# Tamnemng/TAM-GCN

Measured on AMD Instinct MI355X. Metric: skeleton clips/sec (fwd+CE+bwd+grad all-reduce+SGD step), N-UCLA 20-joint x 64-frame, higher is better.
Workload: dtype f32 (exact fp32-input MFMA v_mfma_f32_16x16x4_f32 in every GEMM, forward and backward: the reference's arithmetic); 1 GPU; N-UCLA joint stream, 256 clips/GPU x (3,64,20,1), models.ctrgcn.Model fwd+CE+bwd+grad-allreduce+SGD step, train-mode BN; global_batch=256, streams=1, parallelism=dp1, launch=hipgraph, model_streams=0, rehearsal=False, allreduce=one flat bucket after backward

## Files before the change

### include/tamgcn.h

```cpp
#ifndef TAMGCN_H
#define TAMGCN_H

#ifdef __cplusplus
extern "C" {
#endif

#define TAMGCN_VERSION 401
#define TAMGCN_MAX_SUBSETS 3
#define TAMGCN_MAX_V 32

typedef struct tamgcn_src {
    const float* x1;
    const float* x2;
    const float* coef;
    int ctot;
    int coff;
    int act;
} tamgcn_src;

int         tamgcn_version(void);
const char* tamgcn_last_error(void);
const char* tamgcn_last_kernel(void);
int         tamgcn_get_split_mode(void);
int         tamgcn_set_split_mode(int mode);
// ... 20 lines not shown
    const tamgcn_src* mask;
    const float* aux;
    const float* aux_center;
    int auxctot, auxcoff;
    float* stats_part;
    int stats_ctot, stats_coff;
    const float* post_coef;
    int post_ctot, post_act;
} tamgcn_conv_desc;

int tamgcn_conv_nparts(const tamgcn_conv_desc* d);
int tamgcn_conv(const tamgcn_conv_desc* d, void* stream);

typedef struct tamgcn_wgrad_desc {
    tamgcn_src gy;
    tamgcn_src src;
    int N, M, K, T_in, T_out, V, KT, dil, stride, pad;
    float* part;
    int nsplit;
} tamgcn_wgrad_desc;
int tamgcn_wgrad_max_split(const tamgcn_wgrad_desc* d);
int tamgcn_wgrad(const tamgcn_wgrad_desc* d, void* stream);

typedef struct tamgcn_reduce_desc {
    const float* part; float* out;
    int nsplit, accumulate;
    long long stride_s, count;
    float scale;
} tamgcn_reduce_desc;
int tamgcn_reduce_multi(const tamgcn_reduce_desc* descs, int n, void* stream);

int tamgcn_reduce_sum(float* part, int nsplit, long long stride_s, long long count,
                      float scale, int accumulate, float* out, void* stream);

int tamgcn_bn_fwd_finalize(const float* part, int part_ctot, int part_coff, int nparts, double count,
                           const float* gamma, const float* beta,
                           float* running_mean, float* running_var, long long* num_batches_tracked,
                           float momentum, float eps, int training,
                           float* coef, float* save, int coef_ctot, int coef_coff, int C, void* stream);

int tamgcn_coef_diff(const float* coef_d, const float* coef_y, float* out, int C, int mode, void* stream);

int tamgcn_bn_bwd_finalize(const float* part, int part_ctot, int part_coff, int nparts, double count,
                           const float* gamma, const float* save, int save_ctot, int save_coff,
                           int training, float* dgamma, float* dbeta, float* dbias_conv,
                           float* coef, int coef_ctot, int coef_coff, int C, void* stream);
// ... 222 lines not shown
```

### tam_gcn_amd/_lib.py

```python
import ctypes as C
import os

_HERE = os.path.dirname(os.path.abspath(__file__))
LIB_PATH = os.path.join(_HERE, 'libtamgcn.so')

c_float_p = C.c_void_p


class Src(C.Structure):
    _fields_ = [('x1', C.c_void_p), ('x2', C.c_void_p), ('coef', C.c_void_p),
                ('ctot', C.c_int), ('coff', C.c_int), ('act', C.c_int)]


class ConvDesc(C.Structure):
    _fields_ = [('src', Src),
                ('N', C.c_int), ('K', C.c_int), ('T_in', C.c_int), ('V', C.c_int),
                ('w', C.c_void_p), ('bias', C.c_void_p),
                ('M', C.c_int), ('KT', C.c_int), ('dil', C.c_int), ('stride', C.c_int), ('pad', C.c_int),
                ('wmode', C.c_int), ('up', C.c_int),
                ('y', C.c_void_p), ('yctot', C.c_int), ('ycoff', C.c_int),
                ('T_out', C.c_int), ('T_y', C.c_int), ('ostride', C.c_int),
                ('add1', C.c_void_p), ('add2', C.c_void_p), ('bcast', C.c_void_p), ('bcast_scale', C.c_float),
                ('mask', C.POINTER(Src)),
                ('aux', C.c_void_p), ('aux_center', C.c_void_p), ('auxctot', C.c_int), ('auxcoff', C.c_int),
# ... 1 lines not shown
                ('post_coef', C.c_void_p), ('post_ctot', C.c_int), ('post_act', C.c_int)]


TCONV_MAXB = 6


class TconvDesc(C.Structure):
    _fields_ = [('src', Src),
                ('N', C.c_int), ('T_in', C.c_int), ('T_out', C.c_int), ('V', C.c_int), ('Cb', C.c_int), ('nb', C.c_int),
                ('KT', C.c_int), ('stride', C.c_int), ('pool', C.c_int),
                ('dil', C.c_int * TCONV_MAXB), ('w', C.c_void_p * TCONV_MAXB), ('bias', C.c_void_p * TCONV_MAXB),
                ('y', C.c_void_p), ('yctot', C.c_int), ('ycoff', C.c_int),
                ('stats_part', C.c_void_p), ('stats_ctot', C.c_int),
                ('mask', C.POINTER(Src)), ('center', C.c_void_p)]


class WgradDesc(C.Structure):
    _fields_ = [('gy', Src), ('src', Src),
                ('N', C.c_int), ('M', C.c_int), ('K', C.c_int), ('T_in', C.c_int), ('T_out', C.c_int),
                ('V', C.c_int), ('KT', C.c_int), ('dil', C.c_int), ('stride', C.c_int), ('pad', C.c_int),
                ('part', C.c_void_p), ('nsplit', C.c_int)]


class ReduceDesc(C.Structure):
    _fields_ = [('part', C.c_void_p), ('out', C.c_void_p), ('nsplit', C.c_int), ('accumulate', C.c_int),
                ('stride_s', C.c_longlong), ('count', C.c_longlong), ('scale', C.c_float)]


class BnFwdDesc(C.Structure):
    _fields_ = [('part', C.c_void_p), ('part_ctot', C.c_int), ('part_coff', C.c_int), ('nparts', C.c_int), ('count', C.c_double),
                ('gamma', C.c_void_p), ('beta', C.c_void_p), ('running_mean', C.c_void_p), ('running_var', C.c_void_p),
                ('num_batches_tracked', C.c_void_p), ('momentum', C.c_float), ('eps', C.c_float), ('training', C.c_int),
                ('coef', C.c_void_p), ('save', C.c_void_p), ('coef_ctot', C.c_int), ('coef_coff', C.c_int), ('C', C.c_int)]


class BnBwdDesc(C.Structure):
    _fields_ = [('part', C.c_void_p), ('part_ctot', C.c_int), ('part_coff', C.c_int), ('nparts', C.c_int), ('count', C.c_double),
                ('gamma', C.c_void_p), ('save', C.c_void_p), ('save_ctot', C.c_int), ('save_coff', C.c_int), ('training', C.c_int),
                ('dgamma', C.c_void_p), ('dbeta', C.c_void_p), ('dbias_conv', C.c_void_p), ('coef', C.c_void_p),
                ('coef_ctot', C.c_int), ('coef_coff', C.c_int), ('C', C.c_int)]


class CtrgcDesc(C.Structure):
    _fields_ = [('N', C.c_int), ('Cin', C.c_int), ('Cout', C.c_int), ('S', C.c_int), ('R', C.c_int),
                ('T', C.c_int), ('V', C.c_int),
                ('x', Src),
# ... 25 lines not shown
                ('mode', C.c_int), ('nesterov', C.c_int),
                ('momentum', C.c_float), ('dampening', C.c_float), ('weight_decay', C.c_float), ('eps', C.c_float),
                ('beta1', C.c_double), ('beta2', C.c_double)]


class GradGuard(C.Structure):
    _fields_ = [('max_norm', C.c_float), ('skip_nonfinite', C.c_int), ('partial', C.c_void_p), ('n_partial', C.c_int),
                ('stat', C.c_void_p), ('skipped', C.c_void_p)]


_i, _p, _d, _f, _ll = C.c_int, C.c_void_p, C.c_double, C.c_float, C.c_longlong
_SP = C.POINTER(Src)
SIGNATURES = {
    'tamgcn_version': (_i, []),
    'tamgcn_last_error': (C.c_char_p, []),
    'tamgcn_last_kernel': (C.c_char_p, []),
    'tamgcn_ctrgc_lds_bytes': (_i, [_i, _i, _i]),
    'tamgcn_get_split_mode': (_i, []),
    'tamgcn_set_split_mode': (_i, [_i]),
    'tamgcn_conv_nparts': (_i, [C.POINTER(ConvDesc)]),
    'tamgcn_conv': (_i, [C.POINTER(ConvDesc), _p]),
    'tamgcn_wgrad_max_split': (_i, [C.POINTER(WgradDesc)]),
    'tamgcn_wgrad': (_i, [C.POINTER(WgradDesc), _p]),
    'tamgcn_stem_stats': (_i, [_p, _p, _p, _i, _i, _i, _i, _i, _p, _p]),
    'tamgcn_stem_apply': (_i, [_p, _p, _p, _i, _i, _i, _i, _i, _p, _p]),
    'tamgcn_head_pool_fwd': (_i, [_p, _i, _i, _i, _i, _i, _p, _p]),
    'tamgcn_head_pool_bwd': (_i, [_p, _i, _i, _i, _i, _i, _p, _p]),
    'tamgcn_head_fc_fwd': (_i, [_p, _p, _p, _i, _i, _i, _p, _p]),
    'tamgcn_head_fc_bwd': (_i, [_p, _p, _p, _i, _i, _i, _p, _p, _p, _p]),
    'tamgcn_reduce_multi': (_i, [C.POINTER(ReduceDesc), _i, _p]),
    'tamgcn_reduce_sum': (_i, [_p, _i, _ll, _ll, _f, _i, _p, _p]),
    'tamgcn_bn_fwd_finalize': (_i, [_p, _i, _i, _i, _d, _p, _p, _p, _p, _p, _f, _f, _i, _p, _p, _i, _i, _i, _p]),
    'tamgcn_bn_bwd_finalize': (_i, [_p, _i, _i, _i, _d, _p, _p, _i, _i, _i, _p, _p, _p, _p, _i, _i, _i, _p]),
    'tamgcn_bn_fwd_finalize_multi': (_i, [C.POINTER(BnFwdDesc), _i, _p]),
    'tamgcn_coef_diff': (_i, [_p, _p, _p, _i, _i, _p]),
    'tamgcn_bn_bwd_finalize_multi': (_i, [C.POINTER(BnBwdDesc), _i, _p]),
    'tamgcn_tmean': (_i, [_SP, _i, _i, _i, _i, _p, _p]),
    'tamgcn_ctrgc_build_e': (_i, [C.POINTER(CtrgcDesc), _p, _p]),
    'tamgcn_ctrgc_fwd': (_i, [C.POINTER(CtrgcDesc), _p, _p, _p, _p]),
    'tamgcn_ctrgc_bwd_dx3': (_i, [C.POINTER(CtrgcDesc), _SP, _p, _p, _p]),
    'tamgcn_ctrgc_bwd_de_acc': (_i, [C.POINTER(CtrgcDesc), _SP, _p, _p, _p]),
    'tamgcn_ctrgc_bwd_de_tail': (_i, [C.POINTER(CtrgcDesc), _p, _p, _p, _p, _p, _p, _i, _p]),
    'tamgcn_ctrgc_tiled_supported': (_i, [_i]),
    'tamgcn_ctrgc_tiled_chunks': (_i, [_i]),
    'tamgcn_ctrgc_tiled_build_e': (_i, [C.POINTER(CtrgcDesc), _p, _p]),
    'tamgcn_ctrgc_tiled_agg_fwd': (_i, [C.POINTER(CtrgcDesc), _p, _p, _p, _p, _p]),
# ... 98 lines not shown
```

### tam_gcn_amd/csrc/wgrad.hip

```cpp
#include "common.h"

namespace {

struct WgradArgs {
    SrcDev gy, src;
    int N, M, K, T_in, T_out, V, dil, stride, pad;
    float* part; int nsplit;
    int BT, TIN;
    int PY, PX;
    int n_per;
    int KTG;
};

__device__ __forceinline__ float wg_apply(float x1, float x2, float c1, float c2, float c0, int act) {
    float v = fmaf(c1, x1, fmaf(c2, x2, c0));
    return act == 1 ? fmaxf(v, 0.f) : v;
}

template <bool VEC>
__device__ __forceinline__ void wg_fill(float* tile, int pitch, const float* cf, int rows, int nvalid, int ch0,
                                        const SrcDev& s, long long nbase, long long cs, int T, int V, int f0, int frames) {
    const int tid = threadIdx.x;
    const int len = frames * V;
    if constexpr (VEC) {
        const int l4 = len >> 2;
        for (int e = tid; e < rows * l4; e += NTHREADS) {
            int r = e / l4, c4 = e - r * l4;
            int col = c4 << 2;
            int fr = f0 + col / V;
            float4 o = make_float4(0.f, 0.f, 0.f, 0.f);
            if (r < nvalid && fr >= 0 && fr < T) {
                long long g = nbase + (long long)(ch0 + r) * cs + (long long)f0 * V + col;
                float4 a = *reinterpret_cast<const float4*>(s.x1 + g);
                float4 b = make_float4(0.f, 0.f, 0.f, 0.f);
// ... 243 lines not shown
#pragma unroll
                for (int w = 0; w < 4; ++w) t += smem[(w * KT + tap) * 256 + tid];
                out[((long long)m * a.K + k) * KT + tap] = t;
            }
        }
        return;
    }
#pragma unroll
    for (int tap = 0; tap < KT; ++tap)
#pragma unroll
        for (int x = 0; x < WMT; ++x)
#pragma unroll
            for (int y = 0; y < WKT; ++y)
#pragma unroll
                for (int r = 0; r < 4; ++r) {
                    int m = m0 + (wr * WMT + x) * 16 + kq * 4 + r;
                    int k = k0 + (wc * WKT + y) * 16 + j;
                    if (m < a.M && k < a.K) out[((long long)m * a.K + k) * KT + tap] = acc[tap][x][y][r];
                }
}


constexpr int W_PC = 32, W_NST = 3, W_NT = 512;

template <int WMT, int WKT, int NY, int NX, bool SPL, int NST>
#ifndef TG_WKO
#define TG_WKO 0
#endif
__global__ __launch_bounds__(W_NT, 2) void wgrad_glds_kernel(const WgradArgs a, int ntk, int ntm) {
    extern __shared__ __attribute__((aligned(16))) float smem[];
    constexpr int BMW = 2 * WMT * 16, BKW = 4 * WKT * 16;
    constexpr int RY = BMW * NY, RX = BKW * NX, ROWS = RY + RX;
    constexpr int STG = ROWS * W_PC;
    constexpr int NPIECE = ROWS / 8;
    constexpr int MAXP = (NPIECE + 7) / 8;
    const int tid = threadIdx.x, lane = tid & 63, wave = tid >> 6;
    const int j = lane & 15, kq = lane >> 4, wr = wave >> 2, wc = wave & 3;
    int split, tile, tap;
    {
        const int nt = ntk * ntm, per_tap = nt * a.nsplit;
        int L = blockIdx.x;
        tap = L / per_tap; L -= tap * per_tap;
        if ((a.nsplit & 7) == 0) { const int xcd = L & 7, i = L >> 3; tile = i % nt; split = (i / nt) * 8 + xcd; }
        else { split = L / nt; tile = L - split * nt; }
    }
    const int k0 = (tile % ntk) * BKW, m0 = (tile / ntk) * BMW;
    const long long cs = (long long)a.T_out * a.V;
    const long long csx = (long long)a.T_in * a.V;
// ... 58 lines not shown
        cy0[x] = ok ? a.gy.coef[2 * a.gy.ctot + ch] : 0.f;
    }
#pragma unroll
    for (int y = 0; y < WKT; ++y) {
        const int k = k0 + (wc * WKT + y) * 16 + j;
        const bool ok = k < a.K && a.src.coef;
        const int ch = a.src.coff + (k < a.K ? k : 0);
        cx1[y] = ok ? a.src.coef[ch] : 1.f;
        cx2[y] = (ok && NX == 2) ? a.src.coef[a.src.ctot + ch] : 0.f;
        cx0[y] = ok ? a.src.coef[2 * a.src.ctot + ch] : 0.f;
    }
    const float loy = a.gy.act == 1 ? 0.f : -__builtin_inff(), lox = a.src.act == 1 ? 0.f : -__builtin_inff();
    const bool yplain = !a.gy.coef && a.gy.act != 1, xplain = !a.src.coef && a.src.act != 1;

    f32x4 acc[WMT][WKT];
#pragma unroll
    for (int x = 0; x < WMT; ++x)
#pragma unroll
        for (int y = 0; y < WKT; ++y) acc[x][y] = (f32x4){0.f, 0.f, 0.f, 0.f};

    const int yoff = ((wr * WMT) * 16 + j) * W_PC, xoff = (RY + (wc * WKT) * 16 + j) * W_PC;
    const int sl0 = ((kq) ^ (j & 7)) * 4, sl1 = ((4 + kq) ^ (j & 7)) * 4;

    if (nch > 0) issue(0);
    if (NST == 3 && nch > 1) issue(1);
    for (int c = 0; c < nch; ++c) {
        tg_wait_vmcnt<15>((NST == 3 && c + 1 < nch) ? nissue : 0);
        if (!(TG_WKO & 8)) asm volatile("s_waitcnt lgkmcnt(0)\n\ts_barrier" ::: "memory");
        if (c + NST - 1 < nch) issue(c + NST - 1);
        const float* st = smem + (c % NST) * STG;
        auto frag = [&](int b, f32x4 (&avb)[WMT], f32x4 (&bvb)[WKT]) {
            const int sl = b ? sl1 : sl0;
            if (TG_WKO & 4) {
#pragma unroll
                for (int x = 0; x < WMT; ++x) asm volatile("" : "=v"(avb[x]));
#pragma unroll
                for (int y = 0; y < WKT; ++y) asm volatile("" : "=v"(bvb[y]));
                return;
            }
#pragma unroll
            for (int x = 0; x < WMT; ++x) {
                f32x4 v = *reinterpret_cast<const f32x4*>(st + yoff + x * 16 * W_PC + sl);
                if constexpr (NY == 2) {
                    f32x4 v2 = *reinterpret_cast<const f32x4*>(st + BMW * W_PC + yoff + x * 16 * W_PC + sl);
#pragma unroll
                    for (int e = 0; e < 4; ++e) v[e] = fmaxf(fmaf(cy1[x], v[e], fmaf(cy2[x], v2[e], cy0[x])), loy);
                } else if (!yplain) {
#pragma unroll
                    for (int e = 0; e < 4; ++e) v[e] = fmaxf(fmaf(cy1[x], v[e], cy0[x]), loy);
                }
// ... 24 lines not shown
        f32x4 av[2][WMT], bv[2][WKT];
        frag(0, av[0], bv[0]);
        frag(1, av[1], bv[1]);
        if constexpr (SPL) {
            bf16x8_t ah[WMT], al[WMT], bh[WKT], bl[WKT];
#pragma unroll
            for (int x = 0; x < WMT; ++x) split_bf16x8(av[0][x], av[1][x], ah[x], al[x]);
#pragma unroll
            for (int y = 0; y < WKT; ++y) split_bf16x8(bv[0][y], bv[1][y], bh[y], bl[y]);
#pragma unroll
            for (int y = 0; y < WKT; ++y)
#pragma unroll
                for (int x = 0; x < WMT; ++x) acc[x][y] = mfma_split(ah[x], al[x], bh[y], bl[y], acc[x][y]);
        } else {
#pragma unroll
            for (int b = 0; b < 2; ++b)
#pragma unroll
                for (int e = 0; e < ((TG_WKO & 1) ? (b ? 0 : 1) : 4); ++e)
#pragma unroll
                    for (int y = 0; y < WKT; ++y)
#pragma unroll
                        for (int x = 0; x < WMT; ++x) acc[x][y] = mfma16(av[b][x][e], bv[b][y][e], acc[x][y]);
        }
    }
    float* out = a.part + (long long)split * a.M * a.K * a.KTG + tap;
#pragma unroll
    for (int x = 0; x < WMT; ++x)
#pragma unroll
        for (int y = 0; y < WKT; ++y)
#pragma unroll
            for (int r = 0; r < 4; ++r) {
                const int m = m0 + (wr * WMT + x) * 16 + kq * 4 + r;
                const int k = k0 + (wc * WKT + y) * 16 + j;
                if (m < a.M && k < a.K) out[((long long)m * a.K + k) * a.KTG] = acc[x][y][r];
            }
}

template <int WMT, int WKT, int NY, int NX, bool SPL>
static int launch_wgrad_glds(WgradArgs& a, hipStream_t s) {
    constexpr int BMW = 2 * WMT * 16, BKW = 4 * WKT * 16;
    constexpr size_t STAGE = sizeof(float) * (size_t)(BMW * NY + BKW * NX) * W_PC;
    constexpr int NST = (2 * STAGE <= 80 * 1024 && 3 * STAGE > 80 * 1024) ? 2 : W_NST;
    const size_t lds = NST * STAGE;
    const int ntk = ceil_div(a.K, BKW), ntm = ceil_div(a.M, BMW);
    tg_launch_lds<wgrad_glds_kernel<WMT, WKT, NY, NX, SPL, NST>>(160 * 1024, dim3((unsigned)(ntk * ntm * a.nsplit * a.KTG)), dim3(W_NT), lds, s, a, ntk, ntm);
    tamgcn_note_kernel("wgrad_glds_kernel<%d, %d, %d, %d, %s, %d>%s", WMT, WKT, NY, NX, SPL ? "split" : "f32", NST, a.KTG > 1 ? " taps" : "");
    return 0;
}

template <int WMT, int WKT, bool SPL>
static int launch_wgrad_glds_spl(WgradArgs& a, hipStream_t s) {
    const bool y2 = a.gy.x2 != nullptr, x2 = a.src.x2 != nullptr;
    if (y2 && x2) return launch_wgrad_glds<WMT, WKT, 2, 2, SPL>(a, s);
    if (y2) return launch_wgrad_glds<WMT, WKT, 2, 1, SPL>(a, s);
    if (x2) return launch_wgrad_glds<WMT, WKT, 1, 2, SPL>(a, s);
    return launch_wgrad_glds<WMT, WKT, 1, 1, SPL>(a, s);
}

template <int WMT, int WKT>
static int launch_wgrad_glds_src(WgradArgs& a, hipStream_t s) {
    const int mode = tamgcn_split_mode();
    const bool spl = mode >= 1;
    return spl ? launch_wgrad_glds_spl<WMT, WKT, true>(a, s) : launch_wgrad_glds_spl<WMT, WKT, false>(a, s);
}

static inline int even_pitch(int n) {
    int p = (n + 3) & ~3;
    return p + 2;
}

// ... 64 lines not shown
extern "C" int tamgcn_wgrad_max_split(const tamgcn_wgrad_desc* d) {
    if (!d || d->N <= 0 || d->T_out <= 0 || d->V <= 0) return -1;
    int wmt, wkt;
    if (!wgrad_glds_plan(d, &wmt, &wkt)) {
        const long long m = (long long)d->N * ((d->T_out + 7) / 8);
        return (int)(m < d->N ? d->N : (m > 65535 ? 65535 : m));
    }
    const long long chunks = (long long)d->N * (((long long)(d->T_out - d->pad) * d->V) / W_PC);
    const long long m = chunks / 8;
    return (int)(m < d->N ? d->N : (m > 65535 ? 65535 : m));
}

extern "C" int tamgcn_wgrad(const tamgcn_wgrad_desc* d, void* stream) {
    TG_CHECK(d && d->gy.x1 && d->src.x1 && d->part, "tamgcn_wgrad: null pointer");
    TG_CHECK(d->N > 0 && d->M > 0 && d->K > 0 && d->T_in > 0 && d->T_out > 0 && d->V > 0 && d->nsplit > 0,
             "tamgcn_wgrad: bad dims");
    TG_CHECK(d->gy.coff + d->M <= d->gy.ctot && d->src.coff + d->K <= d->src.ctot, "tamgcn_wgrad: channel slice out of range");
    TG_CHECK(d->nsplit <= tamgcn_wgrad_max_split(d), "tamgcn_wgrad: nsplit=%d exceeds tamgcn_wgrad_max_split=%d", d->nsplit,
             tamgcn_wgrad_max_split(d));
    WgradArgs a;
    a.gy = make_src(d->gy); a.src = make_src(d->src);
    a.N = d->N; a.M = d->M; a.K = d->K; a.T_in = d->T_in; a.T_out = d->T_out; a.V = d->V;
    a.dil = d->dil; a.stride = d->stride; a.pad = d->pad; a.part = d->part; a.nsplit = d->nsplit;
    hipStream_t s = (hipStream_t)stream;
    int rc, wmt, wkt;
    const bool glds = wgrad_glds_plan(d, &wmt, &wkt);
    a.KTG = glds ? d->KT : 1;
    if (glds) {
        if (wmt == 2 && wkt == 2) rc = launch_wgrad_glds_src<2, 1>(a, s);
        else if (wmt == 4 && wkt == 2) rc = launch_wgrad_glds_src<4, 1>(a, s);
        else if (wmt == 2 && wkt == 4) rc = launch_wgrad_glds_src<2, 2>(a, s);
        else rc = launch_wgrad_glds_src<4, 2>(a, s);
        if (rc) return rc;
        TG_LAUNCH_CHECK("tamgcn_wgrad");
        return 0;
    }
    if (d->KT == 1) {
        const int per_row = (d->V + 3) / 4;
        if (wmt == 4 && 128 * per_row > WG_NPF * NTHREADS) wmt = 2;
        if (wkt == 4 && 128 * per_row > WG_NPF * NTHREADS) wkt = 2;
    }
    switch (d->KT) {
        case 1:
            if (wmt == 2 && wkt == 2) rc = launch_wgrad<1, 2, 2>(a, s);
            else if (wmt == 4 && wkt == 2) rc = launch_wgrad<1, 4, 2>(a, s);
            else if (wmt == 2 && wkt == 4) rc = launch_wgrad<1, 2, 4>(a, s);
            else rc = launch_wgrad<1, 4, 4>(a, s);
            break;
        case 3:
            rc = wmt == 1 ? -1 : launch_wgrad<3, 2, 2>(a, s);
            if (rc == -1) rc = launch_wgrad<3, 1, 1>(a, s);
            break;
        case 5:
            rc = (d->M <= 16 && d->K <= 16 && (d->V % 4 == 0 || d->stride == 1)) ? launch_wgrad<5, 1, 1, true>(a, s) : -1;
            if (rc == -1 && wmt != 1) rc = launch_wgrad<5, 2, 2>(a, s);
            if (rc == -1) rc = launch_wgrad<5, 1, 1>(a, s);
            break;
        case 9: rc = launch_wgrad<9, 1, 1>(a, s); break;
        default: tamgcn_set_error("tamgcn_wgrad: kernel size %d not instantiated (1,3,5,9)", d->KT); return -1;
    }
    if (rc) return rc;
    TG_LAUNCH_CHECK("tamgcn_wgrad");
    return 0;
}
```

### tam_gcn_amd/functional.py

```python
import contextlib
import os
import threading

import torch

from . import ops
from .ops import S, RELU


_SIDE = {}
_SIDE_LOCK = threading.Lock()
USE_SIDE_STREAMS = os.environ.get('TAMGCN_SIDE_STREAMS', '1') != '0'

def _side_streams(device, main, k):
    key = (device.index, main.cuda_stream, k)
    got = _SIDE.get(key)
    if got is None:
        with _SIDE_LOCK:
            got = _SIDE.get(key)
            if got is None:
                taken = {main.cuda_stream}
                for (d, m, _), ss in _SIDE.items():
                    if d == device.index:
                        taken.add(m)
# ... 231 lines not shown
                  coef_d=coef_d, save_d=save_d, coef_o=coef_o, save_o=save_o, coef_diff=coef_diff,
                  training=training)
    return g, sv


def gcn_backward(P, sv, dg, need_dx=True, extra_dx=None):
    with ops.ReduceBatch():
        return _gcn_backward(P, sv, dg, need_dx, extra_dx)


def _gcn_backward(P, sv, dg, need_dx=True, extra_dx=None):
    x, xbar, pq, y_pre, d_pre, o_pre, g = sv['x'], sv['xbar'], sv['pq'], sv['y_pre'], sv['d_pre'], sv['o_pre'], sv['g']
    training = sv['training']
    N, Cin, T, V = x.shape
    S_, R, Cout = P.S, P.R, P.Cout
    count = N * T * V
    G = {}
    fk = Fork(x.device, 2)
    fk.__enter__()
    dsum, doz, part_o = ops.gcn_tail_bwd(dg, g, S(o_pre, coef=sv['coef_o']), sv['save_o'])
    coefb_o = torch.empty(3, Cout, device=x.device)
    G['bno.w'], G['bno.b'], G['bo'] = P.bno.bwd(part_o, 0, count, sv['save_o'], 0, training, coefb_o, 0, want_dbias=True)
    gyo = S(doz, o_pre, coefb_o)
    ddiff, _ = ops.conv(gyo, K=Cout, w=P.Wo, bias=None, M=Cout, wmode=1)
    if P.mode == 'conv':
        diff = S(d_pre, y_pre, sv['coef_diff'])
    elif P.mode == 'identity':
        diff = S(x, y_pre, sv['coef_diff'])
    else:
        diff = S(y_pre, None, sv['coef_diff'])
    with fk.on(0):
        G['Wo'] = ops.wgrad(gyo, diff, M=Cout, K=Cout)
    dyb, dres, part2 = ops.gcn_mid_bwd(dsum, ddiff, y_pre, sv['save_y'], d_pre if P.mode == 'conv' else None,
                                       sv['save_d'], want_dres=P.mode != 'zero')
    coefb_y = torch.empty(3, Cout, device=x.device)
    bb = ops.BNBatch()
    G['bn.w'], G['bn.b'], _ = P.bn.bwd(part2, 0, count, sv['save_y'], 0, training, coefb_y, 0, batch=bb)
    coefb_d = None
    if P.mode == 'conv':
        coefb_d = torch.empty(3, Cout, device=x.device)
        G['bnd.w'], G['bnd.b'], G['bd'] = P.bnd.bwd(part2[2:4], 0, count, sv['save_d'], 0, training, coefb_d, 0,
                                                     want_dbias=True, batch=bb)
    bb.flush()
    dy = S(dyb, y_pre, coefb_y)
    xs = S(x)
    cargs = (xs, pq, P.W3, P.B3, P.W4, P.B4, P.PA, P.alpha, Cin, Cout, S_, R, dy)
    fk.refork()
    with fk.on(1):
        G['PA'], G['W4'], G['B4'], G['alpha'], dpq = ops.ctrgc_bwd_de(*cargs, x3=sv['x3'], per_subset=True)
        dpq4 = S(dpq.view(1, S_ * 2 * R, N, V))
        G['W12'] = ops.wgrad(dpq4, S(xbar.view(1, Cin, N, V)), M=S_ * 2 * R, K=Cin, rows=[R] * (2 * S_))
        G['B12'] = dpq.sum((1, 2))
        dxbar = None
        if need_dx:
            dxbar, _ = ops.conv(dpq4, K=S_ * 2 * R, w=P.W12, bias=None, M=Cin, wmode=1)
# ... 227 lines not shown
        if b > 0 and not fused:
            marks.append(fk.mark(b))
        G['bn_in'].append((dgam, dbet))
        dbin.append(dbias)
        if not fused_w:
            with fk.on(b):
                G['Wt'].append(ops.wgrad(gcat(b * Cb), S(h_pre, coef=sv['coef_h'], coff=b * Cb, act=RELU), M=Cb, K=Cb,
                                         KT=k, dil=d, stride=s, pad=pad))
    if fused_w:
        with fk.on(0):
            G['Wt'] = ops.tconv_wgrad(gcat(0), S(h_pre, coef=sv['coef_h'], act=RELU), Cb, P.ks[0], P.dils, s)
    hp = ops.maxpool_bwd(gcat(nb * Cb), S(h_pre, coef=sv['coef_h'], coff=nb * Cb, act=RELU), sv['save_h'], Cb, s, dh,
                         nb * Cb)
    dgam, dbet, dbias = P.bn_in[nb].bwd(hp, nb * Cb, cnt1, sv['save_h'], nb * Cb, training, coefb_h, nb * Cb, True, batch=bi)
    G['bn_in'].append((dgam, dbet))
    dbin.append(dbias)
    for ev in marks:
        fk.wait(ev)
    bi.flush()
    G['bin'] = dbin
    gs = S(g)
    gyh = S(dh, h_pre, coefb_h)
    fk.refork()
    with fk.on(0):
        G['Win'] = ops.wgrad(gyh, gs, M=Ch, K=Cin, rows=[Cb] * (nb + 1))
    with fk.on(1):
        G['Wl'] = ops.wgrad(gcat((nb + 1) * Cb), gs, M=Cb, K=Cin, stride=s)
    dg = None
    if need_dg:
        dg, _ = ops.conv(gyh, K=Ch, w=P.Win, bias=None, M=Cin, wmode=1)
        ops.conv(gcat((nb + 1) * Cb), K=Cb, w=P.Wl, bias=None, M=Cin, wmode=1, y=dg, T_out=T2, ostride=s, add1=dg)
    dxres = None
    if P.rmode == 'identity':
        dxres = dz
    elif P.rmode == 'conv':
        gyr = S(dz, r_pre, coefb_r)
        rk = P.rk
        rpad = (rk - 1) // 2
        fk.refork()
        with fk.on(1):
            G['Wr'] = ops.wgrad(gyr, S(xres), M=Cout, K=xres.shape[1], KT=rk, stride=s, pad=rpad)
        if need_dxres:
            Tx = xres.shape[2]
            if rk == 1:
                dxres = ops.zeros_like(xres) if s > 1 else ops.empty_like(xres)
                ops.conv(gyr, K=Cout, w=P.Wr, bias=None, M=xres.shape[1], wmode=1, y=dxres, T_out=T2, ostride=s)
            else:
                dxres, _ = ops.conv(gyr, K=Cout, w=P.Wr, bias=None, M=xres.shape[1], KT=rk, stride=1,
                                    pad=(rk - 1) - rpad, wmode=1, up=s, T_out=Tx)
    fk.__exit__()
    return dg, dxres, G


# ... 407 lines not shown
```

### tam_gcn_amd/ops.py

```python
import ctypes as C
import os
import threading

import torch

from . import _lib
from ._lib import Src, ConvDesc, WgradDesc, CtrgcDesc, ReduceDesc, TconvDesc, TCONV_MAXB

RELU = 1


def _stream():
    return C.c_void_p(torch.cuda.current_stream().cuda_stream)


def _ptr(t):
    if t is None:
        return None
    if not (t.is_cuda and t.is_contiguous()):
        raise RuntimeError('tam_gcn_amd: expected a contiguous HIP (cuda) tensor; there is no CPU path')
    if t.dtype not in (torch.float32, torch.int64, torch.int32, torch.float64):
        raise RuntimeError(f'tam_gcn_amd: unsupported dtype {t.dtype}')
    return t.data_ptr()


class S:
    __slots__ = ('x1', 'x2', 'coef', 'coff', 'act', 'ctot')

    def __init__(self, x1, x2=None, coef=None, coff=0, act=0):
        self.x1, self.x2, self.coef, self.coff, self.act = x1, x2, coef, coff, act
# ... 186 lines not shown
    nb = len(dils)
    d = TconvDesc()
    d.src = gy.c()
    d.N, d.T_in, d.T_out, d.V, d.Cb, d.nb, d.KT, d.stride = N, T_in, T_out, V, Cb, nb, KT, stride
    for b, dl in enumerate(dils):
        d.dil[b] = int(dl)
    mc = src.c()
    d.mask = C.pointer(mc)
    lib = _lib_()
    mx = lib.tamgcn_tconv_wgrad_max_split(C.byref(d))
    if mx <= 0:
        raise RuntimeError('tamgcn_tconv_wgrad: no tiling for this shape')
    blocks = nb * (1 if Cb == 16 else (Cb // 32) ** 2)
    nsplit = max(1, min(mx, WGRAD_BLOCKS * 2 // blocks))
    part = empty(nsplit, nb, Cb, Cb, KT, like=gy.x1)
    d.y, d.yctot, d.ycoff = _ptr(part), nsplit, 0
    _lib.check(lib.tamgcn_tconv_wgrad(C.byref(d), _stream()), 'tamgcn_tconv_wgrad')
    return reduce_sum(part, nsplit, chunks=[(Cb, Cb, KT, 1)] * nb)


WGRAD_BLOCKS = int(os.environ.get('TAMGCN_WGRAD_BLOCKS', '512'))


def wgrad(gy, src, M, K, KT=1, dil=1, stride=1, pad=0, rows=None):
    N, _, T_out, V = gy.x1.shape
    T_in = src.x1.shape[2]
    per_clip = max(gy.x1.shape[1] * T_out * V, src.x1.shape[1] * T_in * V)
    chunks = n_chunks(N, per_clip) if N * per_clip > CHUNK_ELEMS else [(0, N)]
    taps = KT > 1 and stride == 1 and T_in == T_out and (M > 32 or K > 32 or (V % 4 != 0 and (M > 16 or K > 16)))
    if KT == 1 or taps:
        bm, bk = (64 if M <= 64 else 128), (64 if K <= 64 else 128)
    elif KT == 9:
        bm = bk = 32
    else:
        bm = bk = 32 if (M <= 32 and K <= 32) else 64
    lib = _lib_()
    tiles = ((M + bm - 1) // bm) * ((K + bk - 1) // bk) * (KT if taps else 1)
    descs = []
    for n0, n1 in chunks:
        d = WgradDesc()
        g_, s_ = (gy, src) if len(chunks) == 1 else (_slice_src(gy, n0, n1), _slice_src(src, n0, n1))
        d.gy, d.src = g_.c(), s_.c()
        d.N, d.M, d.K, d.T_in, d.T_out, d.V = n1 - n0, M, K, T_in, T_out, V
        d.KT, d.dil, d.stride, d.pad = KT, dil, stride, pad
        descs.append((d, g_, s_))
    per = max(1, (WGRAD_BLOCKS + tiles - 1) // tiles // len(chunks))
    splits = [max(1, min(lib.tamgcn_wgrad_max_split(C.byref(d)), per)) for d, _, _ in descs]
    nsplit = sum(splits)
    part = empty(nsplit, M, K, KT, like=gy.x1)
    off = 0
    for (d, _, _), ns in zip(descs, splits):
        d.part, d.nsplit = part.data_ptr() + 4 * off * M * K * KT, ns
        _lib.check(lib.tamgcn_wgrad(C.byref(d), _stream()), 'tamgcn_wgrad')
        off += ns
    if rows is not None:
        return reduce_sum(part, nsplit, chunks=[(m, K, KT, 1) for m in rows])
    if nsplit == 1:
        return part.view(M, K, KT, 1)
    return reduce_sum(part, nsplit).view(M, K, KT, 1)


class ReduceBatch:
    _tls = threading.local()

    @staticmethod
    def active():
        return getattr(ReduceBatch._tls, 'active', None)

    def __enter__(self):
        self.items, self.prev = [], ReduceBatch.active()
        ReduceBatch._tls.active = self
        return self

    def __exit__(self, *exc):
        ReduceBatch._tls.active = self.prev
        if self.items and exc[0] is None:
            arr = (ReduceDesc * len(self.items))()
            for i, (part, nsplit, stride, off, count, scale, acc, out) in enumerate(self.items):
                arr[i] = ReduceDesc(part.data_ptr() + 4 * off, _ptr(out), nsplit, int(acc), stride, count, scale)
            _lib.check(_lib_().tamgcn_reduce_multi(arr, len(self.items), _stream()), 'tamgcn_reduce_multi')
        self.items = []
        return False
# ... 625 lines not shown
```

Before: 9224 clips/s.

## Fuse 1x1 conv data gradient into the weight-gradient kernel's LDS stream

Adds a fused wgrad+dx kernel variant. It reuses the gy tiles already staged in LDS for the weight-gradient GEMM to also compute the 1x1 conv input gradient (dx = W^T·act(gy)) with extra MFMAs, and writes dx directly. It is routed by default for the TCN output 1x1 conv and the bottleneck input conv in backward. The goal is to avoid a second pass over gy through a separate conv launch, at the cost of extra registers, LDS and per-stage work in the wgrad kernel. The split count for the fused path defaults to WGRAD_BLOCKS rather than a tile-based count, which may change how the work is split.

```diff
diff --git a/include/tamgcn.h b/include/tamgcn.h
--- a/include/tamgcn.h
+++ b/include/tamgcn.h
@@ -66,6 +66,15 @@
 int tamgcn_wgrad_max_split(const tamgcn_wgrad_desc* d);
 int tamgcn_wgrad(const tamgcn_wgrad_desc* d, void* stream);
 
+typedef struct tamgcn_wgrad_dx_desc {
+    tamgcn_wgrad_desc wg;
+    const float* w;
+    long long ws_m, ws_k;
+    float* dx;
+    int dx_ctot, dx_coff;
+} tamgcn_wgrad_dx_desc;
+int tamgcn_wgrad_dx(const tamgcn_wgrad_dx_desc* d, void* stream);
+
 typedef struct tamgcn_reduce_desc {
     const float* part; float* out;
     int nsplit, accumulate;
diff --git a/tam_gcn_amd/_lib.py b/tam_gcn_amd/_lib.py
--- a/tam_gcn_amd/_lib.py
+++ b/tam_gcn_amd/_lib.py
@@ -47,6 +47,11 @@
                 ('part', C.c_void_p), ('nsplit', C.c_int)]
 
 
+class WgradDxDesc(C.Structure):
+    _fields_ = [('wg', WgradDesc), ('w', C.c_void_p), ('ws_m', C.c_longlong), ('ws_k', C.c_longlong),
+                ('dx', C.c_void_p), ('dx_ctot', C.c_int), ('dx_coff', C.c_int)]
+
+
 class ReduceDesc(C.Structure):
     _fields_ = [('part', C.c_void_p), ('out', C.c_void_p), ('nsplit', C.c_int), ('accumulate', C.c_int),
                 ('stride_s', C.c_longlong), ('count', C.c_longlong), ('scale', C.c_float)]
@@ -118,6 +123,7 @@
     'tamgcn_conv': (_i, [C.POINTER(ConvDesc), _p]),
     'tamgcn_wgrad_max_split': (_i, [C.POINTER(WgradDesc)]),
     'tamgcn_wgrad': (_i, [C.POINTER(WgradDesc), _p]),
+    'tamgcn_wgrad_dx': (_i, [C.POINTER(WgradDxDesc), _p]),
     'tamgcn_stem_stats': (_i, [_p, _p, _p, _i, _i, _i, _i, _i, _p, _p]),
     'tamgcn_stem_apply': (_i, [_p, _p, _p, _i, _i, _i, _i, _i, _p, _p]),
     'tamgcn_head_pool_fwd': (_i, [_p, _i, _i, _i, _i, _i, _p, _p]),
diff --git a/tam_gcn_amd/csrc/wgrad.hip b/tam_gcn_amd/csrc/wgrad.hip
--- a/tam_gcn_amd/csrc/wgrad.hip
+++ b/tam_gcn_amd/csrc/wgrad.hip
@@ -10,6 +10,7 @@
     int PY, PX;
     int n_per;
     int KTG;
+    float* dx; const float* w; long long ws_m, ws_k; int dx_ctot, dx_coff;
 };
 
 __device__ __forceinline__ float wg_apply(float x1, float x2, float c1, float c2, float c0, int act) {
@@ -299,8 +300,9 @@
 
 
 constexpr int W_PC = 32, W_NST = 3, W_NT = 512;
-
-template <int WMT, int WKT, int NY, int NX, bool SPL, int NST>
+typedef f32x4 f32x4_a4 __attribute__((aligned(4)));
+
+template <int WMT, int WKT, int NY, int NX, bool SPL, int NST, bool DX = false>
 #ifndef TG_WKO
 #define TG_WKO 0
 #endif
@@ -405,10 +407,51 @@
     const int yoff = ((wr * WMT) * 16 + j) * W_PC, xoff = (RY + (wc * WKT) * 16 + j) * W_PC;
     const int sl0 = ((kq) ^ (j & 7)) * 4, sl1 = ((4 + kq) ^ (j & 7)) * 4;
 
+    static_assert(!DX || !SPL, "the fused data gradient exists in the exact fp32 form only");
+    constexpr int NPT = DX ? WKT : 1;
+    float wreg[DX ? BMW / 4 : 1];
+    int dx_e[NPT], dx_o[NPT];
+    bool dx_on = false;
+    int dx_nst = 0;
+    long long dx_lane = 0;
+    float* cfd = smem + NST * STG;
+    if constexpr (DX) {
+        const int nkt = a.K >> 4;
+        const int kt = WKT == 2 ? wave : wave % nkt, pt0 = WKT == 2 ? 0 : wave / nkt;
+        dx_on = pt0 < 2;
+        dx_nst = dx_on ? NPT : 0;
+        const int k = kt * 16 + j;
+#pragma unroll
+        for (int s = 0; s < BMW / 4; ++s) {
+            const int m = min(4 * s + kq, a.M - 1);
+            wreg[s] = a.w[(long long)m * a.ws_m + (long long)k * a.ws_k];
+        }
+        const int lb = kq * W_PC + (((j >> 2) ^ kq) << 2) + (j & 3);
+#pragma unroll
+        for (int i = 0; i < NPT; ++i) {
+            const int pt = (pt0 + i) & 1;
+            dx_e[i] = lb + pt * 16; dx_o[i] = lb + (pt ^ 1) * 16;
+        }
+        dx_lane = (long long)(a.dx_coff + k) * cs + ((pt0 & 1) * 16 + 4 * kq);
+        {
+            const int mrow = min(tid, a.M - 1), ch = a.gy.coff + mrow;
+            f32x4 t = {1.f, 0.f, 0.f, 0.f};
+            if (a.gy.coef) {
+                t[0] = a.gy.coef[ch];
+                if (NY == 2) t[1] = a.gy.coef[a.gy.ctot + ch];
+                t[2] = a.gy.coef[2 * a.gy.ctot + ch];
+            }
+            if (tid < a.M) *reinterpret_cast<f32x4*>(cfd + 4 * tid) = t;
+        }
+#pragma unroll
+        for (int s = 0; s < BMW / 4; ++s) asm volatile("" : "+v"(wreg[s]));
+    }
+
     if (nch > 0) issue(0);
     if (NST == 3 && nch > 1) issue(1);
     for (int c = 0; c < nch; ++c) {
-        tg_wait_vmcnt<15>((NST == 3 && c + 1 < nch) ? nissue : 0);
+        if constexpr (DX) tg_wait_vmcnt<15>(((NST == 3 && c + 1 < nch) ? nissue : 0) + dx_nst * min(c, NST - 1));
+        else tg_wait_vmcnt<15>((NST == 3 && c + 1 < nch) ? nissue : 0);
         if (!(TG_WKO & 8)) asm volatile("s_waitcnt lgkmcnt(0)\n\ts_barrier" ::: "memory");
         if (c + NST - 1 < nch) issue(c + NST - 1);
         const float* st = smem + (c % NST) * STG;
@@ -479,6 +522,45 @@
 #pragma unroll
                         for (int x = 0; x < WMT; ++x) acc[x][y] = mfma16(av[b][x][e], bv[b][y][e], acc[x][y]);
         }
+        if constexpr (DX) {
+            if (dx_on) {
+                f32x4 dacc[NPT];
+#pragma unroll
+                for (int i = 0; i < NPT; ++i) dacc[i] = (f32x4){0.f, 0.f, 0.f, 0.f};
+#pragma unroll
+                for (int blk = 0; blk < BMW / 16; ++blk) {
+                    if (blk * 16 < a.M) {
+                        f32x4 cf[4];
+                        float r1[NPT][4], r2[NPT][4];
+#pragma unroll
+                        for (int q = 0; q < 4; ++q) {
+                            const int s = blk * 4 + q;
+                            cf[q] = *reinterpret_cast<const f32x4*>(cfd + (4 * s + kq) * 4);
+#pragma unroll
+                            for (int i = 0; i < NPT; ++i) {
+                                const int o = ((s & 1) ? dx_o[i] : dx_e[i]) + s * 4 * W_PC;
+                                r1[i][q] = st[o];
+                                if constexpr (NY == 2) r2[i][q] = st[BMW * W_PC + o];
+                            }
+                        }
+#pragma unroll
+                        for (int q = 0; q < 4; ++q)
+#pragma unroll
+                            for (int i = 0; i < NPT; ++i) {
+                                float v;
+                                if constexpr (NY == 2) v = fmaxf(fmaf(cf[q][0], r1[i][q], fmaf(cf[q][1], r2[i][q], cf[q][2])), loy);
+                                else v = fmaxf(fmaf(cf[q][0], r1[i][q], cf[q][2]), loy);
+                                dacc[i] = mfma16(v, wreg[blk * 4 + q], dacc[i]);
+                            }
+                    }
+                }
+                const int gc = c_begin + c, nn = gc / cps, pc = gc - nn * cps;
+                const int po = pc < cpf ? pc * W_PC : wlen - W_PC;
+                float* dp = a.dx + (long long)nn * a.dx_ctot * cs + dx_lane + po;
+#pragma unroll
+                for (int i = 0; i < NPT; ++i) *reinterpret_cast<f32x4_a4*>(dp + i * 16) = dacc[i];
+            }
+        }
     }
     float* out = a.part + (long long)split * a.M * a.K * a.KTG + tap;
 #pragma unroll
@@ -493,16 +575,25 @@
             }
 }
 
-template <int WMT, int WKT, int NY, int NX, bool SPL>
+template <int WMT, int WKT, int NY, int NX, bool SPL, bool DX = false>
 static int launch_wgrad_glds(WgradArgs& a, hipStream_t s) {
     constexpr int BMW = 2 * WMT * 16, BKW = 4 * WKT * 16;
     constexpr size_t STAGE = sizeof(float) * (size_t)(BMW * NY + BKW * NX) * W_PC;
     constexpr int NST = (2 * STAGE <= 80 * 1024 && 3 * STAGE > 80 * 1024) ? 2 : W_NST;
-    const size_t lds = NST * STAGE;
+    const size_t lds = NST * STAGE + (DX ? sizeof(float) * 4 * BMW : 0);
     const int ntk = ceil_div(a.K, BKW), ntm = ceil_div(a.M, BMW);
-    tg_launch_lds<wgrad_glds_kernel<WMT, WKT, NY, NX, SPL, NST>>(160 * 1024, dim3((unsigned)(ntk * ntm * a.nsplit * a.KTG)), dim3(W_NT), lds, s, a, ntk, ntm);
-    tamgcn_note_kernel("wgrad_glds_kernel<%d, %d, %d, %d, %s, %d>%s", WMT, WKT, NY, NX, SPL ? "split" : "f32", NST, a.KTG > 1 ? " taps" : "");
+    tg_launch_lds<wgrad_glds_kernel<WMT, WKT, NY, NX, SPL, NST, DX>>(160 * 1024, dim3((unsigned)(ntk * ntm * a.nsplit * a.KTG)), dim3(W_NT), lds, s, a, ntk, ntm);
+    tamgcn_note_kernel("wgrad_glds_kernel<%d, %d, %d, %d, %s, %d>%s%s", WMT, WKT, NY, NX, SPL ? "split" : "f32", NST, a.KTG > 1 ? " taps" : "", DX ? " +dx" : "");
     return 0;
+}
+
+template <int WMT, int WKT>
+static int launch_wgrad_glds_dx(WgradArgs& a, hipStream_t s) {
+    const bool y2 = a.gy.x2 != nullptr, x2 = a.src.x2 != nullptr;
+    if (y2 && x2) return launch_wgrad_glds<WMT, WKT, 2, 2, false, true>(a, s);
+    if (y2) return launch_wgrad_glds<WMT, WKT, 2, 1, false, true>(a, s);
+    if (x2) return launch_wgrad_glds<WMT, WKT, 1, 2, false, true>(a, s);
+    return launch_wgrad_glds<WMT, WKT, 1, 1, false, true>(a, s);
 }
 
 template <int WMT, int WKT, bool SPL>
@@ -613,6 +704,7 @@
     a.gy = make_src(d->gy); a.src = make_src(d->src);
     a.N = d->N; a.M = d->M; a.K = d->K; a.T_in = d->T_in; a.T_out = d->T_out; a.V = d->V;
     a.dil = d->dil; a.stride = d->stride; a.pad = d->pad; a.part = d->part; a.nsplit = d->nsplit;
+    a.dx = nullptr; a.w = nullptr; a.ws_m = a.ws_k = 0; a.dx_ctot = a.dx_coff = 0;
     hipStream_t s = (hipStream_t)stream;
     int rc, wmt, wkt;
     const bool glds = wgrad_glds_plan(d, &wmt, &wkt);
@@ -654,3 +746,37 @@
     TG_LAUNCH_CHECK("tamgcn_wgrad");
     return 0;
 }
+
+extern "C" int tamgcn_wgrad_dx(const tamgcn_wgrad_dx_desc* dd, void* stream) {
+    TG_CHECK(dd && dd->wg.gy.x1 && dd->wg.src.x1 && dd->wg.part && dd->w && dd->dx, "tamgcn_wgrad_dx: null pointer");
+    const tamgcn_wgrad_desc* d = &dd->wg;
+    TG_CHECK(d->N > 0 && d->M > 0 && d->K > 0 && d->T_in > 0 && d->T_out > 0 && d->V > 0 && d->nsplit > 0, "tamgcn_wgrad_dx: bad dims");
+    TG_CHECK(d->KT == 1 && d->stride == 1 && d->pad == 0 && d->T_in == d->T_out, "tamgcn_wgrad_dx: 1x1, stride 1, T_in == T_out only");
+    TG_CHECK(d->M <= 128 && d->M % 16 == 0 && (d->K == 16 || d->K == 32 || d->K == 64 || d->K == 128),
+             "tamgcn_wgrad_dx: M=%d K=%d: needs M <= 128, M %% 16 == 0 and K in {16, 32, 64, 128}", d->M, d->K);
+    TG_CHECK(d->gy.coff >= 0 && d->src.coff >= 0 && d->gy.coff + d->M <= d->gy.ctot && d->src.coff + d->K <= d->src.ctot,
+             "tamgcn_wgrad_dx: channel slice out of range");
+    TG_CHECK(dd->dx_coff >= 0 && dd->dx_coff + d->K <= dd->dx_ctot, "tamgcn_wgrad_dx: dx channel slice out of range");
+    TG_CHECK(tamgcn_split_mode() == 0, "tamgcn_wgrad_dx: exact fp32 GEMM mode only (split mode keeps the two launches)");
+    int wmt, wkt;
+    TG_CHECK(wgrad_glds_plan(d, &wmt, &wkt) && wmt * 32 >= d->M && wkt * 32 >= d->K,
+             "tamgcn_wgrad_dx: no single LDS-DMA tile holds dW for this descriptor (M=%d K=%d, %d+%d sources, T*V=%d)", d->M, d->K,
+             d->gy.x2 ? 2 : 1, d->src.x2 ? 2 : 1, d->T_out * d->V);
+    TG_CHECK(d->nsplit <= tamgcn_wgrad_max_split(d), "tamgcn_wgrad_dx: nsplit=%d exceeds tamgcn_wgrad_max_split=%d", d->nsplit,
+             tamgcn_wgrad_max_split(d));
+    WgradArgs a;
+    a.gy = make_src(d->gy); a.src = make_src(d->src);
+    a.N = d->N; a.M = d->M; a.K = d->K; a.T_in = d->T_in; a.T_out = d->T_out; a.V = d->V;
+    a.dil = d->dil; a.stride = d->stride; a.pad = d->pad; a.part = d->part; a.nsplit = d->nsplit;
+    a.KTG = 1;
+    a.dx = dd->dx; a.w = dd->w; a.ws_m = dd->ws_m; a.ws_k = dd->ws_k; a.dx_ctot = dd->dx_ctot; a.dx_coff = dd->dx_coff;
+    hipStream_t s = (hipStream_t)stream;
+    int rc;
+    if (wmt == 2 && wkt == 2) rc = launch_wgrad_glds_dx<2, 1>(a, s);
+    else if (wmt == 4 && wkt == 2) rc = launch_wgrad_glds_dx<4, 1>(a, s);
+    else if (wmt == 2 && wkt == 4) rc = launch_wgrad_glds_dx<2, 2>(a, s);
+    else rc = launch_wgrad_glds_dx<4, 2>(a, s);
+    if (rc) return rc;
+    TG_LAUNCH_CHECK("tamgcn_wgrad_dx");
+    return 0;
+}
diff --git a/tam_gcn_amd/functional.py b/tam_gcn_amd/functional.py
--- a/tam_gcn_amd/functional.py
+++ b/tam_gcn_amd/functional.py
@@ -277,15 +277,18 @@
     coefb_o = torch.empty(3, Cout, device=x.device)
     G['bno.w'], G['bno.b'], G['bo'] = P.bno.bwd(part_o, 0, count, sv['save_o'], 0, training, coefb_o, 0, want_dbias=True)
     gyo = S(doz, o_pre, coefb_o)
-    ddiff, _ = ops.conv(gyo, K=Cout, w=P.Wo, bias=None, M=Cout, wmode=1)
     if P.mode == 'conv':
         diff = S(d_pre, y_pre, sv['coef_diff'])
     elif P.mode == 'identity':
         diff = S(x, y_pre, sv['coef_diff'])
     else:
         diff = S(y_pre, None, sv['coef_diff'])
-    with fk.on(0):
-        G['Wo'] = ops.wgrad(gyo, diff, M=Cout, K=Cout)
+    if ops.wgrad_dx_routed(gyo, diff, Cout, Cout):
+        G['Wo'], ddiff = ops.wgrad_dx(gyo, diff, M=Cout, K=Cout, w=P.Wo)
+    else:
+        ddiff, _ = ops.conv(gyo, K=Cout, w=P.Wo, bias=None, M=Cout, wmode=1)
+        with fk.on(0):
+            G['Wo'] = ops.wgrad(gyo, diff, M=Cout, K=Cout)
     dyb, dres, part2 = ops.gcn_mid_bwd(dsum, ddiff, y_pre, sv['save_y'], d_pre if P.mode == 'conv' else None,
                                        sv['save_d'], want_dres=P.mode != 'zero')
     coefb_y = torch.empty(3, Cout, device=x.device)
@@ -559,13 +562,18 @@
     gs = S(g)
     gyh = S(dh, h_pre, coefb_h)
     fk.refork()
-    with fk.on(0):
-        G['Win'] = ops.wgrad(gyh, gs, M=Ch, K=Cin, rows=[Cb] * (nb + 1))
+    fused_in = need_dg and ops.wgrad_dx_routed(gyh, gs, Ch, Cin)
+    if not fused_in:
+        with fk.on(0):
+            G['Win'] = ops.wgrad(gyh, gs, M=Ch, K=Cin, rows=[Cb] * (nb + 1))
     with fk.on(1):
         G['Wl'] = ops.wgrad(gcat((nb + 1) * Cb), gs, M=Cb, K=Cin, stride=s)
     dg = None
     if need_dg:
-        dg, _ = ops.conv(gyh, K=Ch, w=P.Win, bias=None, M=Cin, wmode=1)
+        if fused_in:
+            G['Win'], dg = ops.wgrad_dx(gyh, gs, M=Ch, K=Cin, w=P.Win, rows=[Cb] * (nb + 1))
+        else:
+            dg, _ = ops.conv(gyh, K=Ch, w=P.Win, bias=None, M=Cin, wmode=1)
         ops.conv(gcat((nb + 1) * Cb), K=Cb, w=P.Wl, bias=None, M=Cin, wmode=1, y=dg, T_out=T2, ostride=s, add1=dg)
     dxres = None
     if P.rmode == 'identity':
diff --git a/tam_gcn_amd/ops.py b/tam_gcn_amd/ops.py
--- a/tam_gcn_amd/ops.py
+++ b/tam_gcn_amd/ops.py
@@ -5,7 +5,7 @@
 import torch
 
 from . import _lib
-from ._lib import Src, ConvDesc, WgradDesc, CtrgcDesc, ReduceDesc, TconvDesc, TCONV_MAXB
+from ._lib import Src, ConvDesc, WgradDesc, WgradDxDesc, CtrgcDesc, ReduceDesc, TconvDesc, TCONV_MAXB
 
 RELU = 1
 
@@ -238,7 +238,7 @@
 WGRAD_BLOCKS = int(os.environ.get('TAMGCN_WGRAD_BLOCKS', '512'))
 
 
-def wgrad(gy, src, M, K, KT=1, dil=1, stride=1, pad=0, rows=None):
+def wgrad(gy, src, M, K, KT=1, dil=1, stride=1, pad=0, rows=None, nsplit=None):
     N, _, T_out, V = gy.x1.shape
     T_in = src.x1.shape[2]
     per_clip = max(gy.x1.shape[1] * T_out * V, src.x1.shape[1] * T_in * V)
@@ -260,7 +260,7 @@
         d.N, d.M, d.K, d.T_in, d.T_out, d.V = n1 - n0, M, K, T_in, T_out, V
         d.KT, d.dil, d.stride, d.pad = KT, dil, stride, pad
         descs.append((d, g_, s_))
-    per = max(1, (WGRAD_BLOCKS + tiles - 1) // tiles // len(chunks))
+    per = max(1, (WGRAD_BLOCKS + tiles - 1) // tiles // len(chunks)) if nsplit is None else int(nsplit)
     splits = [max(1, min(lib.tamgcn_wgrad_max_split(C.byref(d)), per)) for d, _, _ in descs]
     nsplit = sum(splits)
     part = empty(nsplit, M, K, KT, like=gy.x1)
@@ -269,11 +269,64 @@
         d.part, d.nsplit = part.data_ptr() + 4 * off * M * K * KT, ns
         _lib.check(lib.tamgcn_wgrad(C.byref(d), _stream()), 'tamgcn_wgrad')
         off += ns
+    return _wgrad_result(part, nsplit, M, K, KT, rows)
+
+
+def _wgrad_result(part, nsplit, M, K, KT, rows):
     if rows is not None:
         return reduce_sum(part, nsplit, chunks=[(m, K, KT, 1) for m in rows])
     if nsplit == 1:
         return part.view(M, K, KT, 1)
     return reduce_sum(part, nsplit).view(M, K, KT, 1)
+
+
+WGRAD_DX = os.environ.get('TAMGCN_WGRAD_DX', '1') != '0'
+
+
+def wgrad_dx_supported(gy, src, M, K):
+    N, _, T, V = gy.x1.shape
+    if src.x1.shape[2] != T or M > 128 or M % 16 or K not in (16, 32, 64, 128) or T * V < 64:
+        return False
+    if N * max(gy.x1.shape[1], src.x1.shape[1]) * T * V > CHUNK_ELEMS:
+        return False
+    if any(t is not None and t.data_ptr() % 16 for t in (gy.x1, gy.x2, src.x1, src.x2)):
+        return False
+    rows = (64 if M <= 64 else 128) * (2 if gy.x2 is not None else 1) + (64 if K <= 64 else 128) * (2 if src.x2 is not None else 1)
+    if 4 * 3 * rows * 32 > 160 * 1024:
+        return False
+    return _lib_().tamgcn_get_split_mode() == 0
+
+
+def wgrad_dx_pays(M, K, T, V):
+    return True
+
+
+def wgrad_dx_routed(gy, src, M, K):
+    N, _, T, V = gy.x1.shape
+    return WGRAD_DX and wgrad_dx_pays(M, K, T, V) and wgrad_dx_supported(gy, src, M, K)
+
+
+def wgrad_dx(gy, src, M, K, w, rows=None, dx=None, dxcoff=0, nsplit=None):
+    N, _, T, V = gy.x1.shape
+    if dx is None:
+        dx = empty(N, K, T, V, like=gy.x1)
+    if not (WGRAD_DX and wgrad_dx_supported(gy, src, M, K)):
+        conv(gy, K=M, w=w, bias=None, M=K, wmode=1, y=dx, ycoff=dxcoff)
+        return wgrad(gy, src, M, K, rows=rows, nsplit=nsplit), dx
+    lib = _lib_()
+    d = WgradDxDesc()
+    d.wg.gy, d.wg.src = gy.c(), src.c()
+    d.wg.N, d.wg.M, d.wg.K, d.wg.T_in, d.wg.T_out, d.wg.V = N, M, K, T, T, V
+    d.wg.KT, d.wg.dil, d.wg.stride, d.wg.pad = 1, 1, 1, 0
+    per = WGRAD_BLOCKS if nsplit is None else int(nsplit)
+    ns = max(1, min(lib.tamgcn_wgrad_max_split(C.byref(d.wg)), per))
+    part = empty(ns, M, K, 1, like=gy.x1)
+    d.wg.part, d.wg.nsplit = _ptr(part), ns
+    w2 = w.view(M, K)
+    d.w, d.ws_m, d.ws_k = _ptr(w2), K, 1
+    d.dx, d.dx_ctot, d.dx_coff = _ptr(dx), dx.shape[1], dxcoff
+    _lib.check(lib.tamgcn_wgrad_dx(C.byref(d), _stream()), 'tamgcn_wgrad_dx')
+    return _wgrad_result(part, ns, M, K, 1, rows), dx
 
 
 class ReduceBatch:
```

Result: no change. 9221 clips/s, median of 2 (-0.0%).
